# lucidrains/dreamer4

Measured on AMD Instinct MI355X. Metric: imagined latent steps/sec, higher is better.
Workload: dtype f32; 1 GPU; cfg2 Moving-MNIST-latent shape: dim=512 depth=6 heads=8x64 latents=32x32 spatial=4 registers=8; generate(H+1=16 frames, num_steps=4, time cache) + learn_from_experience(ppo) + clip/AdamW both heads; global_batch=256, per_gpu_batch=256, horizon=15, num_steps=4, parallelism=dp1

## Files before the change

dreamer4_amd/_lib.py:

```python
from __future__ import annotations

import ctypes as C
import os

_HERE = os.path.dirname(os.path.abspath(__file__))
LIB_PATH = os.path.join(_HERE, 'libd4hip.so')

D4_MAX_ACTION_TYPES = 8

GEMM_RMS_ROWSCALE, GEMM_SILU, GEMM_SWIGLU, GEMM_TRANS_A, GEMM_TRANS_B, GEMM_ACCUMULATE = 1, 2, 4, 8, 16, 32


class Config(C.Structure):
    _fields_ = [
        ('dim', C.c_int32), ('dim_latent', C.c_int32), ('num_latent_tokens', C.c_int32), ('depth', C.c_int32),
        ('time_block_every', C.c_int32), ('attn_heads', C.c_int32), ('attn_dim_head', C.c_int32),
        ('attn_softclamp_value', C.c_float),
        ('num_spatial_tokens', C.c_int32), ('num_register_tokens', C.c_int32), ('max_steps', C.c_int32),
        ('num_tasks', C.c_int32), ('num_discrete_action_types', C.c_int32),
        ('num_discrete_actions', C.c_int32 * D4_MAX_ACTION_TYPES), ('num_continuous_actions', C.c_int32),
        ('multi_token_pred_len', C.c_int32),
        ('policy_head_mlp_depth', C.c_int32), ('value_head_mlp_depth', C.c_int32),
        ('terminal_mlp_depth', C.c_int32), ('predict_terminals', C.c_int32),
        ('reward_num_bins', C.c_int32), ('value_num_bins', C.c_int32), ('reward_encoder_type', C.c_int32), ('matmul_bf16', C.c_int32), ('head_mlp_recipe', C.c_int32), ('continuous_beta_param', C.c_int32),
# ... 86 lines not shown
    'd4_euler_step': (_I, [_P, _P, _L, _F, _F, _P]),
    'd4_rollout': (_I, [_P, C.POINTER(RolloutIO), _P]),
    'd4_learn': (_I, [_P, C.POINTER(LearnIO), _P]),
    'd4_adamw_clip': (_I, [_P, _P, _P, _P, _L, _I, _F, _F, _F, _F, _F, _F, _F, _P, _P]),
    'd4_profile_bf16_enable': (_I, [_I]),
    'd4_profile_bf16_read': (_I, [C.POINTER(C.c_double), C.POINTER(C.c_double), C.POINTER(C.c_int64)]),
    'd4_profile_enable': (_I, [_I]),
    'd4_profile_read': (_I, [C.POINTER(C.c_double), C.POINTER(C.c_double), C.POINTER(C.c_int64), _I]),
    'd4_profile_classes': (_I, []),
    'd4_gemm_force_config': (_I, [_I]),
    'd4_debug_switch': (_I, [C.c_char_p, _I]),
    'd4_frame_fused_set': (_I, [_I]),
    'd4_profile_class_name': (C.c_char_p, [_I]),
    'd4_profile_glue_enable': (_I, [_I]),
    'd4_profile_glue_read': (_I, [C.POINTER(C.c_double), C.POINTER(C.c_double), C.POINTER(C.c_int64), _I]),
    'd4_profile_glue_classes': (_I, []),
    'd4_profile_glue_read_flops': (_I, [C.POINTER(C.c_double), _I]),
    'd4_measure_peaks': (_I, [_P, C.c_size_t, C.POINTER(C.c_double), C.POINTER(C.c_double), C.POINTER(C.c_double), _P]),
    'd4_profile_glue_class_name': (C.c_char_p, [_I]),
    'd4_debug_buffer': (_I, [_P, C.c_char_p, C.POINTER(_P)]),
    'd4_gemm': (_I, [_P, _I, _P, _I, _P, _I, _P, _P, _I, _I, _I, _I, _I, _F, _P]),
    'd4_gemm_tn': (_I, [_P, _I, _P, _I, _P, _I, _I, _I, _I, _P, C.c_int64, _I, _I, _P]),
    'd4_gemm_tn_bf16': (_I, [_P, _I, _P, _I, _P, _I, _I, _I, _I, _P, C.c_int64, _I, _P]),
    'd4_gemm_pair': (_I, [_P, _I, _P, _P, _I, _I, _I, _P, _I, _P, _P, _I, _I, _I, _I, _I, _F, _P]),
    'd4_gemm_batched': (_I, [_P, _I, _P, _I, _P, _I, _P, _P, _I, _I, _I, _I, _I, _F, _I, _L, _L, _L, _P]),
    'd4_gemm_bf16': (_I, [_P, _I, _P, _I, _P, _I, _P, _P, _I, _I, _I, _I, _I, _F, _P]),
    'd4_gemm_bf16a': (_I, [_P, _I, _P, _I, _P, _I, _P, _P, _P, _I, _I, _I, _I, _I, _F, _I, _P]),
    'd4_cvt_bf16': (_I, [_P, _P, _L, _P]),
    'd4_gemm_bf16a_compact': (_I, [_P, _I, _P, _I, _P, _I, _P, _P, _P, _I, _I, _I, _I, _I, _F, _P, _P, _I, _I, _I, _I, _I, _I, _P]),
    'd4_gemm_bf16a_batched': (_I, [_P, _I, _P, _I, _P, _I, _P, _P, _P, _I, _I, _I, _I, _I, _F, _I, _L, _L, _L, _I, _P]),
    'd4_cvt_rows_bf16': (_I, [_P, _L, _P, _L, _I, _I, _P]),
    'd4_split_bf16x3': (_I, [_P, _P, _L, _L, _P]),
    'd4_gemm_split': (_I, [_P, _I, _P, _L, _I, _P, _I, _P, _P, _I, _I, _I, _I, _I, _F, _I, _P]),
    'd4_split_f16x2': (_I, [_P, _P, _I, _I, _I, _L, _P, _P]),
    'd4_row_scale_exp': (_I, [_P, _L, _I, _I, _P, _P]),
    'd4_gemm_split2': (_I, [_P, _I, _P, _L, _I, _P, _P, _I, _P, _P, _I, _I, _I, _I, _I, _F, _I, _P, _P]),
    'd4_rmsnorm': (_I, [_P, _I, _P, _P, _I, _I, _I, _F, _P]),
    'd4_small_attn': (_I, [_P, _L, _L] * 4 + [_P] + [_P, _L, _L] * 3 + [_P] + [_I] * 4 + [_F] + [_I] * 6 + [_P]),
    'd4_small_attn_wide': (_I, [_P, _L, _L] * 4 + [_P] + [_P, _L, _L] * 3 + [_P] + [_I] * 4 + [_F] + [_I] * 6 + [_P]),
    'd4_pool_mix': (_I, [_P, _I, _P, _I, _P, _P, _I, _P, _I, _P, _P, _I, _I, _I, _F, _P, _P, _P, _P, _P]),
    'd4_time_attn_decode': (_I, [_P, _I, _P, _I, _P, _P, _P, _P, _I, _P] + [_I] * 8 + [_P, _F, _I, _I, _P]),
    'd4_debug_last_form': (C.c_char_p, [C.c_char_p]),
    'd4_debug_forms': (_I, [C.c_char_p, _I, C.POINTER(C.c_char_p)]),
    'd4_rmsnorm_backward': (_I, [_P, _P, _P, _P, _P, _P, _I, _I, _F, _P]),
    'd4_hl_gauss_scalar': (_I, [_P, _I, _P, _P, _I, _I, _P]),
    'd4_ppo_policy_loss': (_I, [_P, _I, _P, _P, _P, _P, _P, _I, _I, _I, _I, _F, _F, _P, _P, _P, _P]),
    'd4_gae': (_I, [_P, _P, _P, _P, _P, _F, _F, _I, _I, _P, _P]),
    'd4_categorical_sample_logp': (_I, [_P, _I, _P, _I, _P, _I, _I, _F, _P, _P, _P]),
    'd4_hl_gauss_ce': (_I, [_P, _I, _P, _P, _P, _I, _I, _F, _F, _F, _F, _I, _P, _P, _P, _P]),
}

_lib = None


class D4Error(RuntimeError):
    pass


def load():
    global _lib
    if _lib is not None:
        return _lib
    if not os.path.isfile(LIB_PATH):
        raise D4Error(f'{LIB_PATH} is missing: run `python -m dreamer4_amd.build` (hipcc, gfx950). '
                      'There is no CPU fallback for the imagination path.')
    default_table = os.path.join(_HERE, 'gemm_tune_default.txt')
# ... 23 lines not shown
```

dreamer4_amd/csrc/engine.hip:

```cpp
#include "common.h"
#include "engine.h"
#include "prof.h"
#include <math.h>
#include <stdarg.h>
#include <stdio.h>
#include <stdlib.h>
#include <string.h>
#include <memory>

using namespace d4;

namespace d4 {

static constexpr float RMS_EPS = 1.1920928955078125e-07f;

static int round_up(int v, int m) { return (v + m - 1) / m * m; }

int engine_layout(d4_engine* e, bool assign) {
    const d4_config& c = e->c;
    size_t off = 0;
    auto alloc_bytes = [&](size_t bytes) -> char* {
        off = (off + 255) / 256 * 256;
        char* p = assign ? e->ws + off : nullptr;
        off += bytes;
// ... 1386 lines not shown
            d4::SampleArgs sa{};
            sa.term_logit = term_logit; sa.bern_u = io->bern_u + (size_t)f * B;
            sa.terminals = io->terminals; sa.lens = io->lens; sa.B = B; sa.na = 0; sa.frame_index = cur;
            if ((rc = d4::sample_actions_terminals(sa, s))) return rc;
        }
        if ((rc = d4::copy_rows(e->x_lat, n_el, io->latents + (size_t)cur * n_el, T * n_el, B, n_el, s))) return rc;
        if (io->ctx_hist && io->noise_context &&
            (rc = d4::copy_rows(io->noise_context + (size_t)f * B * n_el, n_el, io->ctx_hist + (size_t)cur * n_el, T * n_el, B, n_el, s))) return rc;
    }
    return 0;
}

int d4_profile_bf16_enable(int stride) { d4::gemm_bf16_profile_enable(stride); return 0; }
int d4_profile_bf16_read(double* ms, double* flops, int64_t* count) { return d4::gemm_bf16_profile_read(ms, flops, count); }
int d4_profile_enable(int on) { return d4::gemm_profile_enable(on); }
int d4_profile_read(double* ms, double* flops, int64_t* count, int nclass) { return d4::gemm_profile_read(ms, flops, count, nclass); }
int d4_profile_classes(void) { return d4::gemm_profile_classes(); }
int d4_profile_glue_enable(int mask) { return d4::glue_profile_enable(mask); }
int d4_profile_glue_read(double* ms, double* bytes, int64_t* count, int nclass) { return d4::glue_profile_read(ms, bytes, count, nclass); }
int d4_profile_glue_classes(void) { return d4::GL_N; }
int d4_profile_glue_read_flops(double* flops, int nclass) { return d4::glue_profile_read_flops(flops, nclass); }
const char* d4_profile_glue_class_name(int c) { return d4::glue_class_name(c); }
int d4_frame_fused_set(int mode) { return d4::frame_fused_set(mode); }

int d4_debug_switch(const char* name, int value) {
    int* sw = nullptr;
    if (name && !strcmp(name, "time_attn_fused_append")) sw = &d4::g_time_attn_fused_append;
    else if (name && !strcmp(name, "attn_out_cols")) sw = &d4::g_attn_out_cols;
    else if (name && !strcmp(name, "pool_wide_keys")) sw = &d4::g_pool_wide_keys;
    else if (name && !strcmp(name, "time_attn_tiled")) sw = &d4::g_time_attn_tiled;
    else if (name && !strcmp(name, "space_attn_tiled")) sw = &d4::g_space_attn_tiled;
    else if (name && !strcmp(name, "cross_attn_tiled")) sw = &d4::g_cross_attn_tiled;
    else if (name && !strcmp(name, "small_attn_wide")) sw = &d4::g_small_attn_wide;
    if (!sw) return -1;
    const int old = *sw;
    *sw = value;
    return old;
}
int d4_gemm_force_config(int id) {
    d4::gemm_bf16a_force_config(-1);
    d4::gemm_bf16_force_config(-1);
    const int n_main = d4::gemm_force_config(-1);
    if (id < 0) return n_main;
    if (id >= 500) { d4::gemm_bf16a_force_config(id - 500); return d4::gemm_bf16a_configs(); }
    if (id >= 400) { d4::gemm_force_config(id); return d4::gemm_h2_configs(); }
    if (id >= 300) { d4::gemm_force_config(id); return d4::gemm_x3_configs(); }
    if (id >= 200) return d4::gemm_bf16_force_config(id - 200);
    d4::gemm_force_config(id);
    return id >= 100 ? d4::gemm2_configs() : n_main;
}
const char* d4_profile_class_name(int c) { return d4::gemm_profile_class_name(c); }

int d4_debug_buffer(d4_engine* e, const char* name, float** ptr) {
    D4_REQUIRE(e && name && ptr, "null argument");
    struct { const char* n; float* p; } tbl[] = {
        {"slabs", e->slabs}, {"xpool", e->xpool}, {"xfc", e->xfc}, {"cslabs", e->cslabs}, {"proj0", e->proj0}, {"proj", e->proj}, {"att", e->att},
        {"ffh", e->ffh}, {"pool_q", e->pool_q}, {"pool_kv", e->pool_kv}, {"pool_att", e->pool_att}, {"cq", e->cq},
        {"ckv", e->ckv}, {"catt", e->catt}, {"lkv", e->lkv}, {"latt", e->latt}, {"space", e->space}, {"gs", e->gs},
        {"okv", e->okv}, {"oatt", e->oatt}, {"oproj", e->oproj}, {"pred", e->pred}, {"x_lat", e->x_lat},
        {"cache", e->cache}, {"lin_q", e->lin_q}, {"lin_gate", e->lin_gate}, {"lout_q", e->lout_q},
        {"l_logits", e->l_logits}, {"l_dlogits", e->l_dlogits}, {"l_adv", e->l_adv}, {"l_returns", e->l_returns}, {"l_mask", e->l_mask},
    };
    for (auto& t : tbl) if (!strcmp(t.n, name)) {
        D4_REQUIRE(!e->shadow_only(t.p), "debug buffer '%s' exists only as a bf16 image in this engine (matmul_bf16 = 1)", name);
        *ptr = t.p; return 0;
    }
// ... 14 lines not shown
int d4_gemm_pair(const float* A1, int lda1, const float* W1, float* C1, int ldc1, int M1, int N1, const float* A2, int lda2, const float* W2, float* C2,
                 int ldc2, int M2, int N2, int K, int flags, float rms_eps, void* stream) {
    d4::GemmArgs a{A1, lda1, W1, K, C1, ldc1, nullptr, nullptr, 0, M1, N1, K, flags, rms_eps};
    d4::GemmArgs b{A2, lda2, W2, K, C2, ldc2, nullptr, nullptr, 0, M2, N2, K, flags, rms_eps};
    return d4::gemm_pair(a, b, static_cast<hipStream_t>(stream));
}

int d4_gemm_tn(const float* A, int lda, const float* B, int ldb, float* C, int ldc, int M, int N, int K, float* part, int64_t part_floats,
               int tile_n, int slices, void* stream) {
    return d4::gemm_tn(A, lda, B, ldb, C, ldc, M, N, K, part, (size_t)part_floats, static_cast<hipStream_t>(stream), tile_n, slices);
}

int d4_gemm_batched(const float* A, int lda, const float* W, int ldw, float* C, int ldc, const float* bias,
                    const float* R, int ldr, int M, int N, int K, int flags, float rms_eps, int batch,
                    int64_t strideA, int64_t strideW, int64_t strideC, void* stream) {
    d4::GemmArgs g{A, lda, W, ldw, C, ldc, bias, R, ldr, M, N, K, flags, rms_eps};
    g.batch = batch; g.strideA = strideA; g.strideW = strideW; g.strideC = strideC;
    return d4::gemm(g, static_cast<hipStream_t>(stream));
}

int d4_split_bf16x3(const float* src, uint16_t* dst, int64_t n, int64_t plane_stride, void* stream) {
    D4_REQUIRE(src && dst && n >= 0 && plane_stride >= n && (plane_stride % 8) == 0, "d4_split_bf16x3: bad arguments");
    return d4::split_bf16x3(src, dst, n, plane_stride, static_cast<hipStream_t>(stream));
}
int d4_gemm_split(const float* A, int lda, const uint16_t* W3, int64_t plane_stride, int ldw, float* C, int ldc, const float* bias,
                  const float* R, int ldr, int M, int N, int K, int flags, float rms_eps, int config, void* stream) {
    d4::GemmArgs g{A, lda, reinterpret_cast<const float*>(W3), ldw, C, ldc, bias, R, ldr, M, N, K, flags, rms_eps};
    g.Wb = W3; g.wplane = plane_stride;
    D4_REQUIRE(d4::gemm_x3_applicable(g), "d4_gemm_split: call not supported (M=%d N=%d K=%d flags=%d: K %% 32, ldw %% 8, plane_stride %% 8, 16-byte alignment)", M, N, K, flags);
    if (M == 0) return 0;
    if (config == d4::gemm_x3_configs()) return d4::gemm_x3sk_launch(g, static_cast<hipStream_t>(stream));
    if (config >= 0) return d4::gemm_x3_launch(config, g, static_cast<hipStream_t>(stream));
    return d4::gemm_x3_launch(d4::gemm_x3_heuristic(g), g, static_cast<hipStream_t>(stream));
}
int d4_split_f16x2(const float* src, uint16_t* dst, int rows, int cols, int ld, int64_t plane_stride, float* inv_scale, void* stream) {
    D4_REQUIRE(src && dst && inv_scale && rows >= 0 && cols >= 1 && ld >= cols && (ld % 8) == 0 && plane_stride >= (int64_t)rows * ld && (plane_stride % 8) == 0,
               "d4_split_f16x2: bad arguments");
    return d4::split_f16x2_rows(src, dst, rows, cols, ld, plane_stride, inv_scale, static_cast<hipStream_t>(stream));
}
int d4_row_scale_exp(const float* A, int64_t lda, int rows, int K, int32_t* exp_out, void* stream) {
    D4_REQUIRE(A && exp_out && rows >= 0 && K >= 4 && lda >= K, "d4_row_scale_exp: bad arguments");
    return d4::row_scale_exp(A, lda, rows, K, exp_out, static_cast<hipStream_t>(stream));
}
int d4_gemm_split2(const float* A, int lda, const uint16_t* W2, int64_t plane_stride, int ldw, const float* w_inv_scale, float* C, int ldc, const float* bias,
                   const float* R, int ldr, int M, int N, int K, int flags, float rms_eps, int config, const int32_t* a_exp, void* stream) {
    d4::GemmArgs g{A, lda, reinterpret_cast<const float*>(W2), ldw, C, ldc, bias, R, ldr, M, N, K, flags, rms_eps};
    g.Wb = W2; g.wplane = plane_stride; g.wscale = w_inv_scale; g.aexp = a_exp;
    D4_REQUIRE(d4::gemm_h2_applicable(g), "d4_gemm_split2: call not supported (M=%d N=%d K=%d flags=%d: K %% 32, lda %% 4, ldw %% 8, plane_stride %% 8, 16-byte alignment)", M, N, K, flags);
    if (M == 0) return 0;
    return d4::gemm_h2_launch(config >= 0 ? config : d4::gemm_h2_heuristic(g), g, static_cast<hipStream_t>(stream));
}
int d4_gemm_bf16(const float* A, int lda, const uint16_t* Wb, int ldw, float* C, int ldc, const float* bias,
                 const float* R, int ldr, int M, int N, int K, int flags, float rms_eps, void* stream) {
    d4::GemmArgs g{A, lda, reinterpret_cast<const float*>(Wb), ldw, C, ldc, bias, R, ldr, M, N, K, flags, rms_eps};
    g.Wb = Wb;
    return d4::gemm_bf16(g, static_cast<hipStream_t>(stream));
}

int d4_cvt_bf16(const float* src, uint16_t* dst, int64_t n, void* stream) { return d4::cvt_f32_to_bf16(src, dst, n, static_cast<hipStream_t>(stream)); }

int d4_gemm_bf16a(const uint16_t* Ab, int lda, const uint16_t* Wb, int ldw, float* C, int ldc, uint16_t* Cb, const float* bias, const float* R, int ldr,
                  int M, int N, int K, int flags, float rms_eps, int config, void* stream) {
    d4::GemmArgs g{nullptr, lda, nullptr, ldw, C, ldc, bias, R, ldr, M, N, K, flags, rms_eps};
    g.Ab = Ab; g.Wb = Wb; g.Cb = Cb;
    D4_REQUIRE(d4::gemm_bf16a_applicable(g), "d4_gemm_bf16a: call not supported (K %% 64, lda / ldw %% 8, 16-byte aligned operands)");
    if (config >= 100) { g.group_m = -1; config -= 100; }
// ... 118 lines not shown
```

dreamer4_amd/csrc/gemm_x3sk.hip:

```cpp
#include "common.h"
#include <hip/hip_ext.h>
#include "kernels.h"
#include <type_traits>

namespace d4 {

typedef __bf16 bf16x8 __attribute__((ext_vector_type(8)));


constexpr int SK_BM = 128, SK_BN = 128, SK_WGM = 4, SK_WGN = 2, SK_D = 3;
constexpr int SK_BK = 32, SK_LD = SK_BK + 8, SK_NT = SK_WGM * SK_WGN * 64;
constexpr int SK_G = SK_BK / 8;
constexpr int SK_APL = SK_BM * SK_LD, SK_BPL = SK_BN * SK_LD;
constexpr size_t SK_LDS = (size_t)(2 * 3 * (SK_BM + SK_BN) * SK_LD) * 2 + SK_BM * sizeof(float) + 16;
static_assert(SK_BM * SK_G == SK_NT && SK_BN * SK_G == SK_NT, "one 8-element group of each operand per thread and k-tile");

struct SkArgs {
    GemmArgs p;
    int P, F, R;
    int half;
};

__device__ __forceinline__ void split3(float a, __bf16& h1, __bf16& h2, __bf16& h3) {
    h1 = (__bf16)a;
    const float r = a - (float)h1;
    h2 = (__bf16)r;
    h3 = (__bf16)(r - (float)h2);
}


template <int TNV>
__device__ __forceinline__ void sk_item(const SkArgs& s, const int bm0, const int bn0, __bf16* As, __bf16* Bs, float* rowscale_s) {
    const GemmArgs& p = s.p;
    const int kt0 = 0, kt1 = p.K / SK_BK;
    constexpr int BNV = 64 * TNV;
    const int tid = threadIdx.x, lane = tid & 63;
    const int wave = __builtin_amdgcn_readfirstlane(tid >> 6);
    const int wm = wave / SK_WGN, wn = wave % SK_WGN;
    const int lrow = lane & 31, lhalf = lane >> 5;
    const __bf16* Wb = reinterpret_cast<const __bf16*>(p.Wb);
    const int rowsA = min(SK_BM, p.M - bm0), rowsB = min(BNV, p.N - bn0);
    auto uniform_rsrc = [](const void* base, int64_t bytes) {
        const uint64_t bb = reinterpret_cast<uint64_t>(base);
        const uint32_t lo = __builtin_amdgcn_readfirstlane((uint32_t)bb);
        const uint32_t hi = __builtin_amdgcn_readfirstlane((uint32_t)(bb >> 32));
        const int nb = __builtin_amdgcn_readfirstlane((int)(bytes < 0x7FFFFFFF ? bytes : 0x7FFFFFFF));
        return __builtin_amdgcn_make_buffer_rsrc(reinterpret_cast<void*>(((uint64_t)hi << 32) | lo), 0, nb, 0x00020000);
    };
    const __amdgpu_buffer_rsrc_t rsA = uniform_rsrc(p.A + (int64_t)bm0 * p.lda, ((int64_t)(rowsA - 1) * p.lda + p.K) * 4);
    const int64_t wbytes = ((int64_t)(rowsB - 1) * p.ldw + p.K) * 2;
    const __amdgpu_buffer_rsrc_t rsB0 = uniform_rsrc(Wb + (int64_t)bn0 * p.ldw, wbytes);
    const __amdgpu_buffer_rsrc_t rsB1 = uniform_rsrc(Wb + p.wplane + (int64_t)bn0 * p.ldw, wbytes);
    const __amdgpu_buffer_rsrc_t rsB2 = uniform_rsrc(Wb + 2 * p.wplane + (int64_t)bn0 * p.ldw, wbytes);

    f32x4 ra[SK_D][2];
    f32x4 rb[SK_D][3];
    float ssq0 = 0.f, ssq1 = 0.f;
    using S0 = std::integral_constant<int, 0>;
    using S1 = std::integral_constant<int, 1>;
    using S2 = std::integral_constant<int, 2>;
    const int srow = tid / SK_G, scol = (tid % SK_G) * 8;
    const int browB = TNV == 2 ? srow : (srow & 63);
    const bool b_store = TNV == 2 || srow < 64;
    const uint32_t offA = (uint32_t)((srow * p.lda + scol) * 4), offB = (uint32_t)((browB * p.ldw + scol) * 2);
    auto load_tile = [&](auto set_tag, int k0) {
        constexpr int S = decltype(set_tag)::value;
        ra[S][0] = __builtin_bit_cast(f32x4, __builtin_amdgcn_raw_buffer_load_b128(rsA, offA + (uint32_t)k0 * 4, 0, 0));
        ra[S][1] = __builtin_bit_cast(f32x4, __builtin_amdgcn_raw_buffer_load_b128(rsA, offA + (uint32_t)k0 * 4 + 16, 0, 0));
        rb[S][0] = __builtin_bit_cast(f32x4, __builtin_amdgcn_raw_buffer_load_b128(rsB0, offB + (uint32_t)k0 * 2, 0, 0));
        rb[S][1] = __builtin_bit_cast(f32x4, __builtin_amdgcn_raw_buffer_load_b128(rsB1, offB + (uint32_t)k0 * 2, 0, 0));
        rb[S][2] = __builtin_bit_cast(f32x4, __builtin_amdgcn_raw_buffer_load_b128(rsB2, offB + (uint32_t)k0 * 2, 0, 0));
    };
    auto store_tile = [&](auto set_tag, int buf) {
        constexpr int S = decltype(set_tag)::value;
        __bf16* as = As + buf * 3 * SK_APL + srow * SK_LD + scol;
        __bf16* bs = Bs + buf * 3 * SK_BPL + browB * SK_LD + scol;
        if (b_store) {
            *reinterpret_cast<f32x4*>(bs) = rb[S][0];
            *reinterpret_cast<f32x4*>(bs + SK_BPL) = rb[S][1];
            *reinterpret_cast<f32x4*>(bs + 2 * SK_BPL) = rb[S][2];
        }
        const f32x4 v0 = ra[S][0], v1 = ra[S][1];
        bf16x8 o1, o2, o3;
#pragma unroll
        for (int e = 0; e < 4; ++e) {
            __bf16 h1, h2, h3;
            split3(v0[e], h1, h2, h3); o1[e] = h1; o2[e] = h2; o3[e] = h3;
            split3(v1[e], h1, h2, h3); o1[e + 4] = h1; o2[e + 4] = h2; o3[e + 4] = h3;
        }
        *reinterpret_cast<bf16x8*>(as) = o1;
        *reinterpret_cast<bf16x8*>(as + SK_APL) = o2;
        *reinterpret_cast<bf16x8*>(as + 2 * SK_APL) = o3;
        ssq0 = ssq0 + __builtin_fmaf(v0[3], v0[3], __builtin_fmaf(v0[2], v0[2], __builtin_fmaf(v0[1], v0[1], v0[0] * v0[0])));
        ssq1 = ssq1 + __builtin_fmaf(v1[3], v1[3], __builtin_fmaf(v1[2], v1[2], __builtin_fmaf(v1[1], v1[1], v1[0] * v1[0])));
    };

    f32x16 hi[TNV], lo[TNV];
#pragma unroll
    for (int j = 0; j < TNV; ++j)
#pragma unroll
        for (int e = 0; e < 16; ++e) { hi[j][e] = 0.f; lo[j][e] = 0.f; }

    auto mma = [&](int buf, int ks) {
        const __bf16* as = As + buf * 3 * SK_APL + (wm * 32 + lrow) * SK_LD + lhalf * 8 + ks * 16;
        const __bf16* bs = Bs + buf * 3 * SK_BPL + (wn * TNV * 32 + lrow) * SK_LD + lhalf * 8 + ks * 16;
        bf16x8 af[3], bf[3][TNV];
#pragma unroll
        for (int pl = 0; pl < 3; ++pl) {
            af[pl] = *reinterpret_cast<const bf16x8*>(as + pl * SK_APL);
#pragma unroll
            for (int j = 0; j < TNV; ++j) bf[pl][j] = *reinterpret_cast<const bf16x8*>(bs + pl * SK_BPL + j * 32 * SK_LD);
        }
#define D4_SK_TERM(PA, PB, ACC) \
    _Pragma("unroll") for (int j = 0; j < TNV; ++j) ACC[j] = __builtin_amdgcn_mfma_f32_32x32x16_bf16(af[PA], bf[PB][j], ACC[j], 0, 0, 0);
        D4_SK_TERM(2, 0, lo)
        D4_SK_TERM(0, 0, hi)
        D4_SK_TERM(1, 1, lo)
        D4_SK_TERM(0, 2, lo)
        D4_SK_TERM(1, 0, lo)
        D4_SK_TERM(0, 1, lo)
#undef D4_SK_TERM
    };

    const int nk = kt1 - kt0, kbeg = kt0 * SK_BK;
    const int klast = kbeg + (nk - 1) * SK_BK;
    {
        load_tile(S0{}, kbeg);
        load_tile(S1{}, min(kbeg + SK_BK, klast));
        load_tile(S2{}, min(kbeg + 2 * SK_BK, klast));
        store_tile(S0{}, 0);
        __syncthreads();
        auto k_tile = [&](int kt, auto set_tag, auto store_tag) {
            constexpr int S = decltype(set_tag)::value;
            const int buf = kt & 1;
            load_tile(set_tag, min(kbeg + (kt + SK_D) * SK_BK, klast));
            const bool store = decltype(store_tag)::value || kt + 1 < nk;
            mma(buf, 0);
            if (store) store_tile(std::integral_constant<int, (S + 1) % SK_D>{}, buf ^ 1);
            mma(buf, 1);
            if constexpr (decltype(store_tag)::value) {
                constexpr int NMFMA = 2 * 6 * TNV;
#pragma unroll
                for (int i = 0; i < NMFMA; ++i) {
                    __builtin_amdgcn_sched_group_barrier(0x008, 1, 0);
                    __builtin_amdgcn_sched_group_barrier(0x002, 4 * (3 - TNV), 0);
                    __builtin_amdgcn_sched_group_barrier(0x080, 1, 0);
                    __builtin_amdgcn_sched_group_barrier(0x020, 1, 0);
                }
            }
            __syncthreads();
        };
        using Always = std::true_type;
        using Check = std::false_type;
        const int nfull = (nk - 1) / SK_D;
        int kt = 0;
        for (int t = 0; t < nfull; ++t, kt += SK_D) {
            k_tile(kt, S0{}, Always{});
            k_tile(kt + 1, S1{}, Always{});
            k_tile(kt + 2, S2{}, Always{});
// ... 58 lines not shown
        const float rs = rms ? rowscale_s[lr] : 1.f;
        if (swiglu) {
            if constexpr (TNV == 2) {
                const int gn = bn0 + wn * 64 + lrow;
                if (gn >= p.N) continue;
                float val = hi[0][e] * rs, gate = hi[1][e] * rs;
                if (p.bias) { val += p.bias[gn]; gate += p.bias[gn + 32]; }
                const int on = (gn / 64) * 32 + (gn % 64);
                p.C[(int64_t)gm * p.ldc + on] = val * siluf(gate);
            }
        } else {
#pragma unroll
            for (int j = 0; j < TNV; ++j) {
                const int gn = bn0 + wn * TNV * 32 + j * 32 + lrow;
                if (gn >= p.N) continue;
                float v = hi[j][e] * rs;
                if (p.bias) v += p.bias[gn];
                if (p.flags & GEMM_SILU) v = siluf(v);
                if (p.R) v += p.R[(int64_t)gm * p.ldr + gn];
                if (p.flags & GEMM_ACCUMULATE) v += p.C[(int64_t)gm * p.ldc + gn];
                p.C[(int64_t)gm * p.ldc + gn] = v;
                if (p.C2) {
                    const int ts = gm % p.c2_S;
                    const int keep = p.c2_hi - p.c2_lo;
                    const int rank = (ts >= p.c2_lo && ts < p.c2_hi) ? ts - p.c2_lo : ((p.c2_last && ts == p.c2_S - 1) ? keep : -1);
                    if (rank >= 0) p.C2[((int64_t)(gm / p.c2_S) * (keep + p.c2_last) + rank) * p.ldc2 + gn] = v;
                }
            }
        }
    }
    __syncthreads();
}

__global__ __launch_bounds__(SK_NT, 2) void gemm_x3sk_kernel(SkArgs s) {
    const GemmArgs& p = s.p;
    extern __shared__ __attribute__((aligned(16))) char smem_raw[];
    __bf16* As = reinterpret_cast<__bf16*>(smem_raw);
    __bf16* Bs = As + 2 * 3 * SK_APL;
    float* rowscale_s = reinterpret_cast<float*>(Bs + 2 * 3 * SK_BPL);

    const int b = blockIdx.x;
    const int nbn = (p.N + SK_BN - 1) / SK_BN, nbm = (p.M + SK_BM - 1) / SK_BM;
    const int nk_all = p.K / SK_BK;
    auto tile_of = [&](int tile, int& tm, int& tn) {
        int bid = tile;
        const int nblk = nbm * nbn, nx = 8;
        const int q = nblk / nx, r = nblk % nx, x = bid % nx, o = bid / nx;
        bid = (x < r ? x * (q + 1) : r * (q + 1) + (x - r) * q) + o;
        constexpr int RB = 4;
        const int band = bid / (RB * nbn), j = bid % (RB * nbn);
        const int rows = min(RB, nbm - band * RB);
        tm = band * RB + j % rows; tn = j / rows;
    };
    int tm, tn;
    if (s.half) {
        for (int i = 0; i < s.F; ++i) {
            tile_of(b + i * s.P, tm, tn);
            sk_item<2>(s, tm * SK_BM, tn * SK_BN, As, Bs, rowscale_s);
        }
        const int R8 = (s.R + 7) & ~7;
        if (R8 + s.R <= s.P) {
            const int j = b < s.R ? b : b - R8, half = b < s.R ? 0 : 1;
            if (j >= 0 && j < s.R && (b < s.R || b >= R8)) {
                tile_of(s.F * s.P + j, tm, tn);
                const int bn0 = tn * SK_BN + half * 64;
                if (bn0 < p.N) sk_item<1>(s, tm * SK_BM, bn0, As, Bs, rowscale_s);
            }
            return;
        }
        for (int h = b; h < 2 * s.R; h += s.P) {
            tile_of(s.F * s.P + h / 2, tm, tn);
            const int bn0 = tn * SK_BN + (h & 1) * 64;
            if (bn0 < p.N) sk_item<1>(s, tm * SK_BM, bn0, As, Bs, rowscale_s);
        }
        return;
    }
    for (int i = 0; i < s.F + (b < s.R ? 1 : 0); ++i) {
        tile_of(b + i * s.P, tm, tn);
        sk_item<2>(s, tm * SK_BM, tn * SK_BN, As, Bs, rowscale_s);
    }
}

static std::atomic<int> g_sk_cus[64];

static int sk_cus() {
    int dev = 0;
    if (hipGetDevice(&dev) != hipSuccess) dev = 0;
    std::atomic<int>& c = g_sk_cus[dev & 63];
    int n = c.load(std::memory_order_relaxed);
    if (n == 0) {
        if (hipDeviceGetAttribute(&n, hipDeviceAttributeMultiprocessorCount, dev) != hipSuccess || n <= 0) n = 256;
        c.store(n, std::memory_order_relaxed);
    }
    return n;
}


const char* gemm_x3sk_name() { return "gemm_x3sk_kernel"; }

bool gemm_x3sk_applicable(const GemmArgs& p) {
    return gemm_x3_applicable(p) && p.batch <= 1 && p.M > 0 && (!(p.flags & GEMM_SWIGLU) || (p.N % 64) == 0);
}

bool gemm_x3sk_half_plan(const GemmArgs& p, int* F, int* R, int* P_out) {
    const int P = sk_cus();
    const int T = cdiv(p.M, SK_BM) * cdiv(p.N, SK_BN);
    const int f = T / P, r = T - f * P;
    *F = f; *R = r;
    if (P_out) *P_out = P;
    return r > 0 && 2 * r <= P;
}

bool gemm_x3sk_rule(const GemmArgs& p) {
    if (!gemm_x3sk_applicable(p) || p.M < 1024 || p.N < 512) return false;
    int F, R, P;
    return gemm_x3sk_half_plan(p, &F, &R, &P) && F >= 1 && F <= 3;
}

int gemm_x3sk_launch(const GemmArgs& p, hipStream_t stream, hipEvent_t ea, hipEvent_t eb) {
    D4_REQUIRE(gemm_x3sk_applicable(p), "gemm_x3sk: call not supported (M=%d N=%d K=%d flags=%d batch=%d)", p.M, p.N, p.K, p.flags, p.batch);
    SkArgs a;
    a.p = p;
    a.half = gemm_x3sk_half_plan(p, &a.F, &a.R, &a.P) ? 1 : 0;
    const int T = a.F * a.P + a.R;
    if (T < a.P && !a.half) a.P = T;
    static DeviceOnce attr_set;
    if (attr_set.need()) {
        D4_HIP(hipFuncSetAttribute(reinterpret_cast<const void*>(gemm_x3sk_kernel), hipFuncAttributeMaxDynamicSharedMemorySize, (int)SK_LDS));
        attr_set.done();
    }
    const dim3 grid(a.P), block(SK_NT);
    if (ea) hipExtLaunchKernelGGL(gemm_x3sk_kernel, grid, block, (uint32_t)SK_LDS, stream, ea, eb, 0, a);
    else hipLaunchKernelGGL(gemm_x3sk_kernel, grid, block, SK_LDS, stream, a);
    D4_LAUNCH_CHECK();
    return 0;
}

}
```

dreamer4_amd/csrc/kernels.h:

```cpp
#pragma once
#include <hip/hip_runtime.h>
#include <stdint.h>

namespace d4 {

enum : int {
    GEMM_RMS_ROWSCALE = 1,
    GEMM_SILU = 2,
    GEMM_SWIGLU = 4,
    GEMM_TRANS_A = 8,
    GEMM_TRANS_B = 16,
    GEMM_ACCUMULATE = 32,
};

struct GemmArgs {
    const float* A; int lda;
    const float* W; int ldw;
    float* C; int ldc;
    const float* bias;
    const float* R; int ldr;
    int M, N, K;
    int flags;
    float rms_eps;
    double algo_flops = 0;
// ... 45 lines not shown
int gemm_h2_heuristic(const GemmArgs& p);
bool gemm_h2_takes(const GemmArgs& p);
int gemm_h2_launch(int c, const GemmArgs& p, hipStream_t stream, hipEvent_t ea = nullptr, hipEvent_t eb = nullptr);
int split_f16x2_rows(const float* src, uint16_t* dst, int rows, int cols, int ld, int64_t plane, float* inv_scale, hipStream_t s);
int row_scale_exp(const float* A, int64_t lda, int rows, int K, int* out, hipStream_t s);
bool gemm_x3sk_applicable(const GemmArgs& p);
bool gemm_x3sk_rule(const GemmArgs& p);
const char* gemm_x3sk_name();
int gemm_x3sk_launch(const GemmArgs& p, hipStream_t stream, hipEvent_t ea = nullptr, hipEvent_t eb = nullptr);
bool gemm2_applicable(const GemmArgs& p);
bool gemm2_config_valid(int c, const GemmArgs& p);
int gemm2_configs();
const char* gemm2_config_name(int c);
void gemm2_config_tile(int c, int* bm, int* bn);
int gemm2_launch(int c, const GemmArgs& p, hipStream_t stream, hipEvent_t ea = nullptr, hipEvent_t eb = nullptr);
bool gemm2_ksplit_applicable(const GemmArgs& p);
bool gemm2_ksplit_rule(const GemmArgs& p);
int gemm2_ksplit_launch(const GemmArgs& p, hipStream_t stream, hipEvent_t ea = nullptr, hipEvent_t eb = nullptr);
bool gemm2_pair_config_ok(int c);
bool gemm2_pair_applicable(const GemmArgs& a, const GemmArgs& b);
int gemm2_pair_launch(int c, const GemmArgs& a, const GemmArgs& b, hipStream_t stream, hipEvent_t ea = nullptr, hipEvent_t eb = nullptr);
int gemm_pair(const GemmArgs& a, const GemmArgs& b, hipStream_t stream);
bool gemm_skinny_applicable(const GemmArgs& p);
int gemm_skinny(const GemmArgs& p, hipStream_t stream);
bool gemm_skinny_pair_applicable(const GemmArgs& a, const GemmArgs& b);
int gemm_skinny_pair(const GemmArgs& a, const GemmArgs& b, hipStream_t stream);
int gemm_profile_enable(int on);
bool gemm_profile_active();
int gemm_profile_read(double* ms, double* flops, int64_t* count, int nclass);
int gemm_profile_classes();
extern int g_time_attn_fused_append;
extern int g_pool_wide_keys;
extern int g_attn_out_cols;
extern int g_time_attn_tiled;
extern int g_space_attn_tiled;
extern int g_cross_attn_tiled;
extern int g_small_attn_wide;
int gemm_force_config(int id);
const char* gemm_profile_class_name(int c);

struct SmallAttnArgs {
    const float* q;      int64_t q_group_stride, q_item_stride;
    const float* k;      int64_t k_group_stride, k_item_stride;
    const float* v;      int64_t v_group_stride, v_item_stride;
    const float* gate;   int64_t g_group_stride, g_item_stride;
    const float* k_gamma;
    const float* vres;   int64_t r_group_stride, r_item_stride;
    const float* mix;    int64_t m_group_stride, m_item_stride;
    float* out;          int64_t o_group_stride, o_item_stride;
    int groups, heads, nq, nk;
    float softclamp;
    int mask_special;
    int belief;
    int q_lo = 0, q_hi = 0, q_last = 1;
    int dh = 64;
    uint16_t* out_b = nullptr;
    int wide = 0;
};
int small_attn(const SmallAttnArgs& p, hipStream_t stream);
constexpr int WIDE_ATTN_MAX = 1024;
int wide_attn(const SmallAttnArgs& p, hipStream_t stream, const char** form);

struct PoolMixArgs {
    const float* q; int ldq;
    const float* x; int ldx;
    const float* gate_w;
// ... 150 lines not shown
```

include/d4hip.h:

```cpp
#ifndef D4HIP_H
#define D4HIP_H

#include <stddef.h>
#include <stdint.h>

#ifdef __cplusplus
extern "C" {
#endif

#define D4_MAX_ACTION_TYPES 8
#define D4_MODE_DYNAMICS 0
#define D4_MODE_DECODER 1
#define D4_MODE_ENCODER 2
#define D4_MLP_PRE_RMS 0
#define D4_MLP_POST_LAYER 1
#define D4_BETA_SOFTPLUS_P1 0
#define D4_BETA_EXP_P1 1

typedef struct d4_config {
    int32_t dim, dim_latent, num_latent_tokens, depth, time_block_every;
    int32_t attn_heads, attn_dim_head;
    float attn_softclamp_value;
    int32_t num_spatial_tokens, num_register_tokens, max_steps, num_tasks;
    int32_t num_discrete_action_types;
// ... 132 lines not shown
int d4_measure_peaks(void* scratch, size_t scratch_bytes, double* hbm_copy_gbs, double* mfma_f32_tflops, double* mfma_bf16_tflops, void* stream);

int d4_frame_fused_set(int mode);
int d4_debug_switch(const char* name, int value);
int d4_gemm_force_config(int id);

int d4_debug_buffer(d4_engine* e, const char* name, float** ptr);

int d4_gemm(const float* A, int lda, const float* W, int ldw, float* C, int ldc, const float* bias,
            const float* R, int ldr, int M, int N, int K, int flags, float rms_eps, void* stream);
int d4_gemm_pair(const float* A1, int lda1, const float* W1, float* C1, int ldc1, int M1, int N1, const float* A2, int lda2, const float* W2, float* C2,
                 int ldc2, int M2, int N2, int K, int flags, float rms_eps, void* stream);
int d4_gemm_tn(const float* A, int lda, const float* B, int ldb, float* C, int ldc, int M, int N, int K, float* part, int64_t part_floats,
               int tile_n, int slices, void* stream);
int d4_gemm_tn_bf16(const uint16_t* A, int lda, const uint16_t* B, int ldb, float* C, int ldc, int M, int N, int K, float* part, int64_t part_floats,
                    int slices, void* stream);
int d4_gemm_batched(const float* A, int lda, const float* W, int ldw, float* C, int ldc, const float* bias,
                    const float* R, int ldr, int M, int N, int K, int flags, float rms_eps, int batch,
                    int64_t strideA, int64_t strideW, int64_t strideC, void* stream);
int d4_gemm_bf16(const float* A, int lda, const uint16_t* Wb, int ldw, float* C, int ldc, const float* bias,
                 const float* R, int ldr, int M, int N, int K, int flags, float rms_eps, void* stream);
int d4_gemm_bf16a(const uint16_t* Ab, int lda, const uint16_t* Wb, int ldw, float* C, int ldc, uint16_t* Cb, const float* bias, const float* R, int ldr,
                  int M, int N, int K, int flags, float rms_eps, int config, void* stream);
int d4_cvt_bf16(const float* src, uint16_t* dst, int64_t n, void* stream);
int d4_gemm_bf16a_compact(const uint16_t* Ab, int lda, const uint16_t* Wb, int ldw, float* C, int ldc, uint16_t* Cb, const float* bias, const float* R, int ldr,
                          int M, int N, int K, int flags, float rms_eps, float* C2, uint16_t* C2b, int ldc2, int c2_S, int c2_lo, int c2_hi, int c2_last,
                          int config, void* stream);
int d4_gemm_bf16a_batched(const uint16_t* Ab, int lda, const uint16_t* Wb, int ldw, float* C, int ldc, uint16_t* Cb, const float* bias, const float* R, int ldr,
                          int M, int N, int K, int flags, float rms_eps, int batch, int64_t strideA, int64_t strideW, int64_t strideC, int config, void* stream);
int d4_cvt_rows_bf16(const float* src, int64_t lds, uint16_t* dst, int64_t ldd, int rows, int cols, void* stream);
int d4_split_bf16x3(const float* src, uint16_t* dst, int64_t n, int64_t plane_stride, void* stream);
int d4_gemm_split(const float* A, int lda, const uint16_t* W3, int64_t plane_stride, int ldw, float* C, int ldc, const float* bias,
                  const float* R, int ldr, int M, int N, int K, int flags, float rms_eps, int config, void* stream);
int d4_split_f16x2(const float* src, uint16_t* dst, int rows, int cols, int ld, int64_t plane_stride, float* inv_scale, void* stream);
int d4_row_scale_exp(const float* A, int64_t lda, int rows, int K, int32_t* exp_out, void* stream);
int d4_gemm_split2(const float* A, int lda, const uint16_t* W2, int64_t plane_stride, int ldw, const float* w_inv_scale, float* C, int ldc, const float* bias,
                   const float* R, int ldr, int M, int N, int K, int flags, float rms_eps, int config, const int32_t* a_exp, void* stream);
size_t d4_ff_workspace_bytes(int rows, int dim, int inner);
int d4_train_arith_set(int arith);
int d4_train_arith_get(void);
int d4_train_wide_set(int on);
int d4_train_scratch_bind(void* scratch, size_t bytes);
size_t d4_ff_bf16_scratch_bytes(int rows, int dim, int inner);
size_t d4_attn_bf16_scratch_bytes(int rows, int dim, int heads, int dim_head);
size_t d4_cross_attn_bf16_scratch_bytes(int groups, int nq, int nk, int dim, int dim_ctx, int heads, int dim_head);
int d4_ff_forward(const float* x, const float* norm_w, const float* w_in, const float* b_in, const float* w_out, const float* b_out,
                  int rows, int dim, int inner, float* y, float* workspace, size_t workspace_bytes, void* stream);
int d4_ff_backward(const float* x, const float* dy, const float* norm_w, const float* w_in, const float* b_in, const float* w_out,
                   int rows, int dim, int inner, float* dx, float* d_norm_w, float* d_w_in, float* d_b_in, float* d_w_out, float* d_b_out,
                   float* workspace, size_t workspace_bytes, void* stream);
int d4_ff_backward_saved(const float* x, const float* dy, const float* norm_w, const float* w_in, const float* b_in, const float* w_out,
                   int rows, int dim, int inner, float* dx, float* d_norm_w, float* d_w_in, float* d_b_in, float* d_w_out, float* d_b_out,
                   float* workspace, size_t workspace_bytes, void* stream);
size_t d4_attn_workspace_bytes(int frames, int tokens, int dim, int heads, int dim_head);
int d4_space_attn_forward(const float* x, const float* residual_values, const float* norm_w, const float* wq, const float* wk, const float* wv,
                          const float* wo, const float* w_gates, const float* w_mix, const float* b_mix, const float* k_gamma,
                          int frames, int tokens, int dim, int heads, int dim_head, float softclamp, int num_special, int belief,
                          float* y, float* workspace, size_t workspace_bytes, void* stream);
int d4_space_attn_backward(const float* x, const float* residual_values, const float* dy, const float* norm_w, const float* wq, const float* wk,
                           const float* wv, const float* wo, const float* w_gates, const float* w_mix, const float* b_mix, const float* k_gamma,
                           int frames, int tokens, int dim, int heads, int dim_head, float softclamp, int num_special, int belief,
                           float* dx, float* d_residual_values, float* d_norm_w, float* d_wq, float* d_wk, float* d_wv, float* d_wo,
                           float* d_w_gates, float* d_w_mix, float* d_b_mix, float* d_k_gamma,
                           float* workspace, size_t workspace_bytes, void* stream);
int d4_space_attn_backward_saved(const float* x, const float* residual_values, const float* dy, const float* norm_w, const float* wq, const float* wk,
                           const float* wv, const float* wo, const float* w_gates, const float* w_mix, const float* b_mix, const float* k_gamma,
// ... 76 lines not shown
```

Baseline: 21500 imagined steps/s.

## Prefetch LDS fragments one k-tile ahead in split-bf16x3 stream-K GEMM

Adds a variant of the stream-K split-bf16x3 GEMM inner loop that double-buffers LDS, reads MFMA fragments for both k-halves before issuing the next global load, and interleaves split/LDS writes with MFMAs through scheduling group barriers. Register prefetch depth drops from three to two stages. The new variant is the default, with the old path kept behind a debug switch. The aim is to hide LDS and global latency behind MFMA work, at the cost of higher register pressure and a schedule that is sensitive to tuning. It also exposes a compact-output entry point for the split GEMM.

Result: slower. 21270 imagined steps/s (-1.1%).

```diff
diff --git a/dreamer4_amd/_lib.py b/dreamer4_amd/_lib.py
--- a/dreamer4_amd/_lib.py
+++ b/dreamer4_amd/_lib.py
@@ -142,6 +142,7 @@
     'd4_cvt_rows_bf16': (_I, [_P, _L, _P, _L, _I, _I, _P]),
     'd4_split_bf16x3': (_I, [_P, _P, _L, _L, _P]),
     'd4_gemm_split': (_I, [_P, _I, _P, _L, _I, _P, _I, _P, _P, _I, _I, _I, _I, _I, _F, _I, _P]),
+    'd4_gemm_split_compact': (_I, [_P, _I, _P, _L, _I, _P, _I, _P, _P, _I, _I, _I, _I, _I, _F, _P, _I, _I, _I, _I, _I, _I, _P]),
     'd4_split_f16x2': (_I, [_P, _P, _I, _I, _I, _L, _P, _P]),
     'd4_row_scale_exp': (_I, [_P, _L, _I, _I, _P, _P]),
     'd4_gemm_split2': (_I, [_P, _I, _P, _L, _I, _P, _P, _I, _P, _P, _I, _I, _I, _I, _I, _F, _I, _P, _P]),
diff --git a/dreamer4_amd/csrc/engine.hip b/dreamer4_amd/csrc/engine.hip
--- a/dreamer4_amd/csrc/engine.hip
+++ b/dreamer4_amd/csrc/engine.hip
@@ -1442,6 +1442,7 @@
     else if (name && !strcmp(name, "space_attn_tiled")) sw = &d4::g_space_attn_tiled;
     else if (name && !strcmp(name, "cross_attn_tiled")) sw = &d4::g_cross_attn_tiled;
     else if (name && !strcmp(name, "small_attn_wide")) sw = &d4::g_small_attn_wide;
+    else if (name && !strcmp(name, "x3sk_frag_ahead")) sw = &d4::g_x3sk_frag_ahead;
     if (!sw) return -1;
     const int old = *sw;
     *sw = value;
@@ -1522,6 +1523,19 @@
     if (config == d4::gemm_x3_configs()) return d4::gemm_x3sk_launch(g, static_cast<hipStream_t>(stream));
     if (config >= 0) return d4::gemm_x3_launch(config, g, static_cast<hipStream_t>(stream));
     return d4::gemm_x3_launch(d4::gemm_x3_heuristic(g), g, static_cast<hipStream_t>(stream));
+}
+int d4_gemm_split_compact(const float* A, int lda, const uint16_t* W3, int64_t plane_stride, int ldw, float* C, int ldc, const float* bias,
+                          const float* R, int ldr, int M, int N, int K, int flags, float rms_eps, float* C2, int ldc2, int c2_S, int c2_lo, int c2_hi,
+                          int c2_last, int config, void* stream) {
+    d4::GemmArgs g{A, lda, reinterpret_cast<const float*>(W3), ldw, C, ldc, bias, R, ldr, M, N, K, flags, rms_eps};
+    g.Wb = W3; g.wplane = plane_stride;
+    g.C2 = C2; g.ldc2 = ldc2; g.c2_S = c2_S; g.c2_lo = c2_lo; g.c2_hi = c2_hi; g.c2_last = c2_last;
+    D4_REQUIRE(d4::gemm_x3_applicable(g) && !(flags & d4::GEMM_SWIGLU) && C2 && ldc2 >= N && c2_S >= 1 && 0 <= c2_lo && c2_lo <= c2_hi && c2_hi <= c2_S,
+               "d4_gemm_split_compact: call not supported (M=%d N=%d K=%d flags=%d c2_S=%d rows %d..%d)", M, N, K, flags, c2_S, c2_lo, c2_hi);
+    if (M == 0) return 0;
+    if (config == d4::gemm_x3_configs()) return d4::gemm_x3sk_launch(g, static_cast<hipStream_t>(stream));
+    D4_REQUIRE(config >= 0 && config < d4::gemm_x3_configs(), "d4_gemm_split_compact: config %d", config);
+    return d4::gemm_x3_launch(config, g, static_cast<hipStream_t>(stream));
 }
 int d4_split_f16x2(const float* src, uint16_t* dst, int rows, int cols, int ld, int64_t plane_stride, float* inv_scale, void* stream) {
     D4_REQUIRE(src && dst && inv_scale && rows >= 0 && cols >= 1 && ld >= cols && (ld % 8) == 0 && plane_stride >= (int64_t)rows * ld && (plane_stride % 8) == 0,
diff --git a/dreamer4_amd/csrc/gemm_x3sk.hip b/dreamer4_amd/csrc/gemm_x3sk.hip
--- a/dreamer4_amd/csrc/gemm_x3sk.hip
+++ b/dreamer4_amd/csrc/gemm_x3sk.hip
@@ -8,7 +8,7 @@
 typedef __bf16 bf16x8 __attribute__((ext_vector_type(8)));
 
 
-constexpr int SK_BM = 128, SK_BN = 128, SK_WGM = 4, SK_WGN = 2, SK_D = 3;
+constexpr int SK_BM = 128, SK_BN = 128, SK_WGM = 4, SK_WGN = 2, SK_D = 3, SK_D_FA = 2;
 constexpr int SK_BK = 32, SK_LD = SK_BK + 8, SK_NT = SK_WGM * SK_WGN * 64;
 constexpr int SK_G = SK_BK / 8;
 constexpr int SK_APL = SK_BM * SK_LD, SK_BPL = SK_BN * SK_LD;
@@ -29,8 +29,9 @@
 }
 
 
-template <int TNV>
+template <int TNV, bool FA>
 __device__ __forceinline__ void sk_item(const SkArgs& s, const int bm0, const int bn0, __bf16* As, __bf16* Bs, float* rowscale_s) {
+    constexpr int D = FA ? SK_D_FA : SK_D;
     const GemmArgs& p = s.p;
     const int kt0 = 0, kt1 = p.K / SK_BK;
     constexpr int BNV = 64 * TNV;
@@ -53,8 +54,8 @@
     const __amdgpu_buffer_rsrc_t rsB1 = uniform_rsrc(Wb + p.wplane + (int64_t)bn0 * p.ldw, wbytes);
     const __amdgpu_buffer_rsrc_t rsB2 = uniform_rsrc(Wb + 2 * p.wplane + (int64_t)bn0 * p.ldw, wbytes);
 
-    f32x4 ra[SK_D][2];
-    f32x4 rb[SK_D][3];
+    f32x4 ra[D][2];
+    f32x4 rb[D][3];
     float ssq0 = 0.f, ssq1 = 0.f;
     using S0 = std::integral_constant<int, 0>;
     using S1 = std::integral_constant<int, 1>;
@@ -95,6 +96,30 @@
         ssq1 = ssq1 + __builtin_fmaf(v1[3], v1[3], __builtin_fmaf(v1[2], v1[2], __builtin_fmaf(v1[1], v1[1], v1[0] * v1[0])));
     };
 
+    bf16x8 o1, o2, o3;
+    auto split_tile = [&](auto set_tag) {
+        constexpr int S = decltype(set_tag)::value;
+        const f32x4 v0 = ra[S][0], v1 = ra[S][1];
+#pragma unroll
+        for (int e = 0; e < 4; ++e) {
+            __bf16 h1, h2, h3;
+            split3(v0[e], h1, h2, h3); o1[e] = h1; o2[e] = h2; o3[e] = h3;
+            split3(v1[e], h1, h2, h3); o1[e + 4] = h1; o2[e + 4] = h2; o3[e + 4] = h3;
+        }
+        ssq0 = ssq0 + __builtin_fmaf(v0[3], v0[3], __builtin_fmaf(v0[2], v0[2], __builtin_fmaf(v0[1], v0[1], v0[0] * v0[0])));
+        ssq1 = ssq1 + __builtin_fmaf(v1[3], v1[3], __builtin_fmaf(v1[2], v1[2], __builtin_fmaf(v1[1], v1[1], v1[0] * v1[0])));
+    };
+    auto write_tile = [&](auto set_tag, int buf) {
+        constexpr int S = decltype(set_tag)::value;
+        __bf16* as = As + buf * 3 * SK_APL + srow * SK_LD + scol;
+        __bf16* bs = Bs + buf * 3 * SK_BPL + browB * SK_LD + scol;
+        *reinterpret_cast<f32x4*>(bs) = rb[S][0];
+        *reinterpret_cast<f32x4*>(bs + SK_BPL) = rb[S][1];
+        *reinterpret_cast<f32x4*>(bs + 2 * SK_BPL) = rb[S][2];
+        *reinterpret_cast<bf16x8*>(as) = o1;
+        *reinterpret_cast<bf16x8*>(as + SK_APL) = o2;
+        *reinterpret_cast<bf16x8*>(as + 2 * SK_APL) = o3;
+    };
     f32x16 hi[TNV], lo[TNV];
 #pragma unroll
     for (int j = 0; j < TNV; ++j)
@@ -122,9 +147,86 @@
 #undef D4_SK_TERM
     };
 
+    bf16x8 fa[2][3], fb[2][3][TNV];
+    auto frag_read = [&](int buf, auto ks_tag) {
+        constexpr int KS = decltype(ks_tag)::value;
+        const __bf16* as = As + buf * 3 * SK_APL + (wm * 32 + lrow) * SK_LD + lhalf * 8 + KS * 16;
+        const __bf16* bs = Bs + buf * 3 * SK_BPL + (wn * TNV * 32 + lrow) * SK_LD + lhalf * 8 + KS * 16;
+        fa[KS][2] = *reinterpret_cast<const bf16x8*>(as + 2 * SK_APL);
+#pragma unroll
+        for (int j = 0; j < TNV; ++j) fb[KS][0][j] = *reinterpret_cast<const bf16x8*>(bs + j * 32 * SK_LD);
+        fa[KS][0] = *reinterpret_cast<const bf16x8*>(as);
+        fa[KS][1] = *reinterpret_cast<const bf16x8*>(as + SK_APL);
+#pragma unroll
+        for (int j = 0; j < TNV; ++j) fb[KS][1][j] = *reinterpret_cast<const bf16x8*>(bs + SK_BPL + j * 32 * SK_LD);
+#pragma unroll
+        for (int j = 0; j < TNV; ++j) fb[KS][2][j] = *reinterpret_cast<const bf16x8*>(bs + 2 * SK_BPL + j * 32 * SK_LD);
+    };
+    auto mma_frag = [&](auto ks_tag) {
+        constexpr int KS = decltype(ks_tag)::value;
+#define D4_SK_TERM(PA, PB, ACC) \
+    _Pragma("unroll") for (int j = 0; j < TNV; ++j) ACC[j] = __builtin_amdgcn_mfma_f32_32x32x16_bf16(fa[KS][PA], fb[KS][PB][j], ACC[j], 0, 0, 0);
+        D4_SK_TERM(2, 0, lo)
+        D4_SK_TERM(0, 0, hi)
+        D4_SK_TERM(1, 1, lo)
+        D4_SK_TERM(0, 2, lo)
+        D4_SK_TERM(1, 0, lo)
+        D4_SK_TERM(0, 1, lo)
+#undef D4_SK_TERM
+    };
+
     const int nk = kt1 - kt0, kbeg = kt0 * SK_BK;
     const int klast = kbeg + (nk - 1) * SK_BK;
-    {
+    if constexpr (FA) {
+        load_tile(S0{}, kbeg);
+        load_tile(S1{}, min(kbeg + SK_BK, klast));
+        split_tile(S0{});
+        write_tile(S0{}, 0);
+        __syncthreads();
+        auto k_tile = [&](int kt, auto set_tag, auto store_tag) {
+            constexpr int S = decltype(set_tag)::value;
+            using Next = std::integral_constant<int, (S + 1) % D>;
+            const int buf = kt & 1;
+            constexpr int NM = 6 * TNV;
+            frag_read(buf, S0{});
+            load_tile(set_tag, min(kbeg + (kt + D) * SK_BK, klast));
+            frag_read(buf, S1{});
+            __builtin_amdgcn_sched_barrier(0);
+            const bool store = decltype(store_tag)::value || kt + 1 < nk;
+            if (store) split_tile(Next{});
+            mma_frag(S0{});
+            if constexpr (decltype(store_tag)::value) {
+                __builtin_amdgcn_sched_group_barrier(0x002, 24, 0);
+#pragma unroll
+                for (int i = 0; i < NM; ++i) {
+                    __builtin_amdgcn_sched_group_barrier(0x008, 1, 0);
+                    __builtin_amdgcn_sched_group_barrier(0x002, 4 * (3 - TNV), 0);
+                }
+            }
+            __builtin_amdgcn_sched_barrier(0);
+            if (store) write_tile(Next{}, buf ^ 1);
+            mma_frag(S1{});
+            if constexpr (decltype(store_tag)::value) {
+#pragma unroll
+                for (int i = 0; i < 6; ++i) {
+                    __builtin_amdgcn_sched_group_barrier(0x008, 1, 0);
+                    __builtin_amdgcn_sched_group_barrier(0x200, 1, 0);
+                }
+            }
+            __builtin_amdgcn_sched_barrier(0);
+            __syncthreads();
+        };
+        using Always = std::true_type;
+        using Check = std::false_type;
+        const int nfull = (nk - 1) / D;
+        int kt = 0;
+        for (int t = 0; t < nfull; ++t, kt += D) {
+            k_tile(kt, S0{}, Always{});
+            k_tile(kt + 1, S1{}, Always{});
+        }
+        k_tile(kt, S0{}, Check{});
+        if (kt + 1 < nk) k_tile(kt + 1, S1{}, Check{});
+    } else {
         load_tile(S0{}, kbeg);
         load_tile(S1{}, min(kbeg + SK_BK, klast));
         load_tile(S2{}, min(kbeg + 2 * SK_BK, klast));
@@ -249,7 +351,8 @@
     __syncthreads();
 }
 
-__global__ __launch_bounds__(SK_NT, 2) void gemm_x3sk_kernel(SkArgs s) {
+template <bool FA>
+__device__ __forceinline__ void sk_body(const SkArgs& s) {
     const GemmArgs& p = s.p;
     extern __shared__ __attribute__((aligned(16))) char smem_raw[];
     __bf16* As = reinterpret_cast<__bf16*>(smem_raw);
@@ -273,7 +376,7 @@
     if (s.half) {
         for (int i = 0; i < s.F; ++i) {
             tile_of(b + i * s.P, tm, tn);
-            sk_item<2>(s, tm * SK_BM, tn * SK_BN, As, Bs, rowscale_s);
+            sk_item<2, FA>(s, tm * SK_BM, tn * SK_BN, As, Bs, rowscale_s);
         }
         const int R8 = (s.R + 7) & ~7;
         if (R8 + s.R <= s.P) {
@@ -281,22 +384,27 @@
             if (j >= 0 && j < s.R && (b < s.R || b >= R8)) {
                 tile_of(s.F * s.P + j, tm, tn);
                 const int bn0 = tn * SK_BN + half * 64;
-                if (bn0 < p.N) sk_item<1>(s, tm * SK_BM, bn0, As, Bs, rowscale_s);
+                if (bn0 < p.N) sk_item<1, FA>(s, tm * SK_BM, bn0, As, Bs, rowscale_s);
             }
             return;
         }
         for (int h = b; h < 2 * s.R; h += s.P) {
             tile_of(s.F * s.P + h / 2, tm, tn);
             const int bn0 = tn * SK_BN + (h & 1) * 64;
-            if (bn0 < p.N) sk_item<1>(s, tm * SK_BM, bn0, As, Bs, rowscale_s);
+            if (bn0 < p.N) sk_item<1, FA>(s, tm * SK_BM, bn0, As, Bs, rowscale_s);
         }
         return;
     }
     for (int i = 0; i < s.F + (b < s.R ? 1 : 0); ++i) {
         tile_of(b + i * s.P, tm, tn);
-        sk_item<2>(s, tm * SK_BM, tn * SK_BN, As, Bs, rowscale_s);
-    }
-}
+        sk_item<2, FA>(s, tm * SK_BM, tn * SK_BN, As, Bs, rowscale_s);
+    }
+}
+
+__global__ __launch_bounds__(SK_NT, 2) void gemm_x3sk_kernel(SkArgs s) { sk_body<true>(s); }
+__global__ __launch_bounds__(SK_NT, 2) void gemm_x3sk_jit_kernel(SkArgs s) { sk_body<false>(s); }
+
+int g_x3sk_frag_ahead = 1;
 
 static std::atomic<int> g_sk_cus[64];
 
@@ -344,11 +452,13 @@
     static DeviceOnce attr_set;
     if (attr_set.need()) {
         D4_HIP(hipFuncSetAttribute(reinterpret_cast<const void*>(gemm_x3sk_kernel), hipFuncAttributeMaxDynamicSharedMemorySize, (int)SK_LDS));
+        D4_HIP(hipFuncSetAttribute(reinterpret_cast<const void*>(gemm_x3sk_jit_kernel), hipFuncAttributeMaxDynamicSharedMemorySize, (int)SK_LDS));
         attr_set.done();
     }
     const dim3 grid(a.P), block(SK_NT);
-    if (ea) hipExtLaunchKernelGGL(gemm_x3sk_kernel, grid, block, (uint32_t)SK_LDS, stream, ea, eb, 0, a);
-    else hipLaunchKernelGGL(gemm_x3sk_kernel, grid, block, SK_LDS, stream, a);
+    auto kernel = g_x3sk_frag_ahead != 0 ? gemm_x3sk_kernel : gemm_x3sk_jit_kernel;
+    if (ea) hipExtLaunchKernelGGL(kernel, grid, block, (uint32_t)SK_LDS, stream, ea, eb, 0, a);
+    else hipLaunchKernelGGL(kernel, grid, block, SK_LDS, stream, a);
     D4_LAUNCH_CHECK();
     return 0;
 }
diff --git a/dreamer4_amd/csrc/kernels.h b/dreamer4_amd/csrc/kernels.h
--- a/dreamer4_amd/csrc/kernels.h
+++ b/dreamer4_amd/csrc/kernels.h
@@ -101,6 +101,7 @@
 extern int g_time_attn_fused_append;
 extern int g_pool_wide_keys;
 extern int g_attn_out_cols;
+extern int g_x3sk_frag_ahead;
 extern int g_time_attn_tiled;
 extern int g_space_attn_tiled;
 extern int g_cross_attn_tiled;
diff --git a/include/d4hip.h b/include/d4hip.h
--- a/include/d4hip.h
+++ b/include/d4hip.h
@@ -188,6 +188,9 @@
 int d4_split_bf16x3(const float* src, uint16_t* dst, int64_t n, int64_t plane_stride, void* stream);
 int d4_gemm_split(const float* A, int lda, const uint16_t* W3, int64_t plane_stride, int ldw, float* C, int ldc, const float* bias,
                   const float* R, int ldr, int M, int N, int K, int flags, float rms_eps, int config, void* stream);
+int d4_gemm_split_compact(const float* A, int lda, const uint16_t* W3, int64_t plane_stride, int ldw, float* C, int ldc, const float* bias,
+                          const float* R, int ldr, int M, int N, int K, int flags, float rms_eps, float* C2, int ldc2, int c2_S, int c2_lo, int c2_hi,
+                          int c2_last, int config, void* stream);
 int d4_split_f16x2(const float* src, uint16_t* dst, int rows, int cols, int ld, int64_t plane_stride, float* inv_scale, void* stream);
 int d4_row_scale_exp(const float* A, int64_t lda, int rows, int K, int32_t* exp_out, void* stream);
 int d4_gemm_split2(const float* A, int lda, const uint16_t* W2, int64_t plane_stride, int ldw, const float* w_inv_scale, float* C, int ldc, const float* bias,
```
